# yungselm/multimoda-rs

Measured on AMD Instinct MI355X. Metric: Hausdorff pose-evals/sec (frames x poses) for 4-phase full align; best-pose match, higher is better.
Workload: dtype f16 hi+lo matrix-pipe screen (fp32 accumulate) + f64 exact re-score

## Files before the change

### multimoda-rs_amd/csrc/mm_kernels.hip

```cpp

#include <hip/hip_runtime.h>
#include <algorithm>
#include <cstdlib>
#include <type_traits>
#include <vector>
#include <cstdio>

#include "mm_device.h"
#include "mm_screen_limits.h"
#include "mm_xcd.h"
#include "../../include/mm_hausdorff.h"

namespace mm {

typedef float v2f __attribute__((ext_vector_type(2)));

template <typename T> struct Tr;
template <> struct Tr<float> {
    using U = unsigned int;
    using T2 = float2;
    static __device__ __forceinline__ U bits(float v) { return __float_as_uint(v); }
    static __device__ __forceinline__ float from(U u) { return __uint_as_float(u); }
    static __device__ __forceinline__ float inf() { return __uint_as_float(0x7f800000u); }
    static constexpr U INF_BITS = 0x7f800000u;
// ... 477 lines not shown
        }
    }
}


typedef _Float16 h2v __attribute__((ext_vector_type(2)));
typedef float f2v __attribute__((ext_vector_type(2)));

static __device__ __forceinline__ h4v mx_col_coords(float X, float Y)
{
    asm volatile("" : "+v"(X), "+v"(Y));
    h2v h = __builtin_convertvector(f2v{X, Y}, h2v);
    unsigned hb = __builtin_bit_cast(unsigned, h);
    asm volatile("" : "+v"(hb));
    h = __builtin_bit_cast(h2v, hb);
    const h2v l = __builtin_convertvector(f2v{X - (float)h.x, Y - (float)h.y}, h2v);
    return h4v{h.x, h.y, l.x, l.y};
}

static __device__ __forceinline__ h4v mx_col_norm(float X, float Y)
{
    const float n2 = __builtin_fmaf(X, X, Y * Y);
    const _Float16 nh = (_Float16)(n2 * 0.00390625f);
    const _Float16 nl = (_Float16)__builtin_fmaf(-256.0f, (float)nh, n2);
    return h4v{(_Float16)256.0f, (_Float16)1.0f, nh, nl};
}

template <int CTRL>
static __device__ __forceinline__ int dpp_max_i32(int v)
{
    const int o = __builtin_amdgcn_update_dpp((int)0x80000000, v, CTRL, 0xF, 0xF, false);
    return o > v ? o : v;
}
static __device__ __forceinline__ int wave_max_i32_dpp(int v)
{
    v = dpp_max_i32<0xB1>(v); v = dpp_max_i32<0x4E>(v); v = dpp_max_i32<0x141>(v); v = dpp_max_i32<0x140>(v);
    const int r0 = __builtin_amdgcn_readlane(v, 0), r1 = __builtin_amdgcn_readlane(v, 16);
    const int r2 = __builtin_amdgcn_readlane(v, 32), r3 = __builtin_amdgcn_readlane(v, 48);
    const int a = r0 > r1 ? r0 : r1, c = r2 > r3 ? r2 : r3;
    return a > c ? a : c;
}

#ifndef MM_MX_DUAL_MAX
#define MM_MX_DUAL_MAX 5
#endif
template <int NCT, bool CARRY>
static __device__ __forceinline__ int mx_main(unsigned vB, unsigned vA, unsigned vRW, unsigned vRR, int nloop, int tail, unsigned vRS)
{
    if constexpr (NCT <= MM_MX_DUAL_MAX) return MxMainD<NCT, CARRY>::run(vB, vA, nloop, tail, vRS);
    else return MxMain<NCT, CARRY>::run(vB, vA, vRW, vRR, 0u, nloop, tail, vRS);
}
template <int NCT>
static __device__ __forceinline__ int mx_emit(unsigned vB, unsigned vA, unsigned vRW, unsigned vRR, int nloop, int tail, unsigned vRS,
                                              unsigned vCS)
{
    if constexpr (NCT <= MM_MX_DUAL_MAX) return MxEmitD<NCT>::run(vB, vA, nloop, tail, vRS, vCS);
    else return MxEmit<NCT>::run(vB, vA, vRW, vRR, 0u, nloop, tail, vRS, vCS);
}

static __device__ __forceinline__ unsigned wave_min_u32_dpp(unsigned v)
{
    return ~(unsigned)wave_max_i32_dpp((int)~(v ^ 0x80000000u)) ^ 0x80000000u;
}

template <int NCT, bool MULTI, int WAVES = 4>
__global__ void __launch_bounds__(64 * WAVES, 2)
k_screen_mx(const PairDesc* __restrict__ pairs, const WorkItem* __restrict__ work, int n_work_host,
            const int* __restrict__ n_work_dev, const int32_t* __restrict__ sel, int a_cap, const float* __restrict__ ptx,
            const float* __restrict__ pty, const float* __restrict__ cosv, const float* __restrict__ sinv, float* __restrict__ out_sq)
{
    constexpr int NB = NCT * 32;
    constexpr int NQ = (NCT + 1) / 2;
    extern __shared__ __align__(16) unsigned char smem[];
    h8v* s_a = reinterpret_cast<h8v*>(smem);
    h4v* s_bw = reinterpret_cast<h4v*>(s_a + a_cap * 64);
    int* s_redx = reinterpret_cast<int*>(s_bw + WAVES * NCT * 64);
    int* s_rsx = s_redx + WAVES * MX_RED;
    float* s_cs = reinterpret_cast<float*>(s_rsx + (MULTI ? WAVES * a_cap * 32 : 0));
    int* s_ci = reinterpret_cast<int*>(s_cs + 2 * MX_ITEM);

    const int tid = threadIdx.x, lane = tid & 63, wave = tid >> 6, l32 = lane & 31, hi = lane >> 5;
    h4v* s_b = s_bw + wave * NCT * 64;
    int* s_rs = s_rsx + wave * a_cap * 32;
    const unsigned lds0 = (unsigned)(size_t)smem;
    const unsigned vB = lds0 + (unsigned)((size_t)s_b - (size_t)smem) + lane * 8;
    const unsigned vA = lds0 + (unsigned)((size_t)s_a - (size_t)smem) + lane * 16;
    const unsigned red_w = lds0 + (unsigned)((size_t)s_redx - (size_t)smem) + wave * MX_RED * 4;
    const unsigned vRW = red_w + (hi * 16) * MM_SCREEN_MX_RED_STRIDE + l32 * 4;
    const int rh = (l32 >> 2) & 1, rv = (l32 & 3) + 4 * (l32 >> 3);
    const unsigned vRR = red_w + (rh * 16 + rv) * MM_SCREEN_MX_RED_STRIDE + hi * 64;
    const unsigned vRS = lds0 + (unsigned)((size_t)s_rs - (size_t)smem) + l32 * 4;
    const int n_work = n_work_dev ? *n_work_dev : n_work_host;

    for (int wi = (int)gridDim.x == n_work ? xcd_work_index(blockIdx.x, n_work) : (int)blockIdx.x; wi < n_work;
         wi += gridDim.x) {
        const WorkItem w = work[wi];
        const PairDesc pd = pairs[w.pair];
        const int na = pd.n_ref, nb = pd.n_tgt;
        const int nrt = (na + 31) >> 5;
        const int nloop = (nrt - 1) >> 1, tail = (nrt - 1) & 1;
        const float S = __builtin_ldexpf(1.0f, pd.pad0), inv_s2 = __builtin_ldexpf(1.0f, -2 * pd.pad0);

        __syncthreads();
        for (int t = tid; t < 2 * w.cnt; t += 64 * WAVES) {
            const int a = sel ? sel[pd.out_off + w.a0 + (t >> 1)] : w.a0 + (t >> 1);
            s_cs[t] = (t & 1) ? sinv[pd.tab_off + a] : cosv[pd.tab_off + a];
            if (!(t & 1)) s_ci[t >> 1] = a;
        }
        mx_stage_rows<64 * WAVES>(s_a, nrt, na, ptx + pd.ref_off, pty + pd.ref_off, S, tid);
        if constexpr (!MULTI) {
            float tx[NQ], ty[NQ];
#pragma unroll
            for (int q = 0; q < NQ; ++q) {
                const int j = lane + 64 * q;
                const int jc = j < nb ? j : nb - 1;
                tx[q] = S * ptx[pd.tgt_off + jc]; ty[q] = S * pty[pd.tgt_off + jc];
                if (j < NB) s_b[(j >> 5) * 64 + (j & 31) + 32] = mx_col_norm(tx[q], ty[q]);
            }
            __syncthreads();

            for (int k = wave; k < w.cnt; k += WAVES) {
                const float c = s_cs[2 * k], s = s_cs[2 * k + 1];
                const int a = s_ci[k];
#pragma unroll
                for (int q = 0; q < NQ; ++q) {
                    const int j = lane + 64 * q;
                    if (j < NB) {
                        const float bx = __builtin_fmaf(tx[q], c, -(ty[q] * s));
                        const float by = __builtin_fmaf(tx[q], s, ty[q] * c);
                        s_b[(j >> 5) * 64 + (j & 31)] = mx_col_coords(bx, by);
                    }
                }
                int m = mx_main<NCT, false>(vB, vA, vRW, vRR, nloop, tail, vRS);
                m = wave_max_i32_dpp(m);
                if (lane == 0) out_sq[pd.out_off + a] = __int_as_float(m) * inv_s2;
            }
        } else {
            __syncthreads();
            const int nblk = (((nb + 31) >> 5) + NCT - 1) / NCT;
            for (int k = wave; k < w.cnt; k += WAVES) {
                const float c = s_cs[2 * k], s = s_cs[2 * k + 1];
                const int a = s_ci[k];
                for (int i = lane; i < nrt * 32; i += 64) s_rs[i] = 0x7f800000;
                int m = 0;
                for (int blk = 0; blk < nblk; ++blk) {
#pragma unroll
                    for (int q = 0; q < NQ; ++q) {
                        const int j = lane + 64 * q;
                        if (j < NB) {
                            const int jg = blk * NB + j;
                            const int jc = jg < nb ? jg : nb - 1;
                            const float x = S * ptx[pd.tgt_off + jc], y = S * pty[pd.tgt_off + jc];
                            const float bx = __builtin_fmaf(x, c, -(y * s));
                            const float by = __builtin_fmaf(x, s, y * c);
                            s_b[(j >> 5) * 64 + (j & 31) + 32] = mx_col_norm(x, y);
                            s_b[(j >> 5) * 64 + (j & 31)] = mx_col_coords(bx, by);
                        }
                    }
                    const int mb = mx_main<NCT, true>(vB, vA, vRW, vRR, nloop, tail, vRS);
                    m = mb > m ? mb : m;
                }
                for (int i = lane; i < nrt * 32; i += 64) { const int r = s_rs[i]; m = r > m ? r : m; }
                m = wave_max_i32_dpp(m);
                if (lane == 0) out_sq[pd.out_off + a] = __int_as_float(m) * inv_s2;
            }
        }
    }
}

template <int NCT>
__global__ void __launch_bounds__(64, 2)
k_screen_mx_emit(const PairDesc* __restrict__ pairs, const WorkItem* __restrict__ work, const int* __restrict__ n_work_dev, int a_cap,
                 const float* __restrict__ ptx, const float* __restrict__ pty, const float* __restrict__ cosv,
                 const float* __restrict__ sinv, float* __restrict__ out_sq, float* __restrict__ emit, int emit_rows, int emit_cols)
{
    constexpr int NB = NCT * 32, NQ = (NCT + 1) / 2;
    extern __shared__ __align__(16) unsigned char smem[];
    h8v* s_a = reinterpret_cast<h8v*>(smem);
    h4v* s_b = reinterpret_cast<h4v*>(s_a + a_cap * 64);
    int* s_red = reinterpret_cast<int*>(s_b + NCT * 64);
    int* s_rs = s_red + MX_RED;
    int* s_col = s_rs + a_cap * 32;
    const int lane = threadIdx.x, l32 = lane & 31, hi = lane >> 5;
    const unsigned lds0 = (unsigned)(size_t)smem;
    const unsigned vB = lds0 + (unsigned)((size_t)s_b - (size_t)smem) + lane * 8;
    const unsigned vA = lds0 + lane * 16;
    const unsigned red_w = lds0 + (unsigned)((size_t)s_red - (size_t)smem);
    const unsigned vRW = red_w + (hi * 16) * MM_SCREEN_MX_RED_STRIDE + l32 * 4;
    const int rh = (l32 >> 2) & 1, rv = (l32 & 3) + 4 * (l32 >> 3);
    const unsigned vRR = red_w + (rh * 16 + rv) * MM_SCREEN_MX_RED_STRIDE + hi * 64;
    const unsigned vRS = lds0 + (unsigned)((size_t)s_rs - (size_t)smem) + l32 * 4;
    const unsigned vCS = lds0 + (unsigned)((size_t)s_col - (size_t)smem) + lane * 4;
    const int n_work = *n_work_dev;

    for (int wi = blockIdx.x; wi < n_work; wi += gridDim.x) {
        const WorkItem w = work[wi];
        const PairDesc pd = pairs[w.pair];
        const int na = pd.n_ref, nb = pd.n_tgt, a = w.a0;
        const int nrt = (na + 31) >> 5, nloop = (nrt - 1) >> 1, tail = (nrt - 1) & 1;
        const float S = __builtin_ldexpf(1.0f, pd.pad0), inv_s2 = __builtin_ldexpf(1.0f, -2 * pd.pad0);
        const float c = cosv[pd.tab_off + a], s = sinv[pd.tab_off + a];
        __syncthreads();
        mx_stage_rows<64>(s_a, nrt, na, ptx + pd.ref_off, pty + pd.ref_off, S, lane);
        for (int i = lane; i < nrt * 32; i += 64) s_rs[i] = 0x7f800000;
#pragma unroll
        for (int q = 0; q < NQ; ++q) {
            const int j = lane + 64 * q;
            if (j < NB) {
                const int jc = j < nb ? j : nb - 1;
                const float x = S * ptx[pd.tgt_off + jc], y = S * pty[pd.tgt_off + jc];
                s_b[(j >> 5) * 64 + (j & 31) + 32] = mx_col_norm(x, y);
                s_b[(j >> 5) * 64 + (j & 31)] = mx_col_coords(__builtin_fmaf(x, c, -(y * s)), __builtin_fmaf(x, s, y * c));
            }
        }
        __syncthreads();
        int m = mx_emit<NCT>(vB, vA, vRW, vRR, nloop, tail, vRS, vCS);
        __syncthreads();
        float* const em = emit + (size_t)w.pair * (size_t)(emit_rows + emit_cols);
        for (int i = lane; i < nrt * 32; i += 64) {
            const int r = s_rs[i];
            m = r > m ? r : m;
            if (i < na) em[i] = __int_as_float(r) * inv_s2;
        }
        for (int j = lane; j < nb; j += 64) em[emit_rows + j] = __int_as_float(s_col[j]) * inv_s2;
        m = wave_max_i32_dpp(m);
        if (lane == 0) out_sq[pd.out_off + a] = __int_as_float(m) * inv_s2;
    }
}

template <int NCT>
static hipError_t launch_mx_emit_t(const BatchDev& b, const WorkItem* work, const int* n_dev, int cap, int a_cap, hipStream_t s)
{
    const size_t lds = (size_t)a_cap * 64 * 16 + (size_t)NCT * 64 * 8 + (size_t)MX_RED * 4 + (size_t)a_cap * 32 * 4 +
                       (size_t)((NCT + 1) / 2) * 64 * 4;
    hipError_t e = hipFuncSetAttribute(reinterpret_cast<const void*>(k_screen_mx_emit<NCT>), hipFuncAttributeMaxDynamicSharedMemorySize, (int)lds);
    if (e != hipSuccess) return e;
    hipLaunchKernelGGL((k_screen_mx_emit<NCT>), dim3(std::min(cap, 256 * 8 * 2)), dim3(64), lds, s, b.pairs, work, n_dev, a_cap, b.p32x,
                       b.p32y, b.cos32, b.sin32, b.sq32, b.emit, b.emit_rows, b.emit_cols);
    return hipGetLastError();
}

static hipError_t launch_mx_emit(const BatchDev& b, const WorkItem* work, const int* n_dev, int cap, int nct, int a_cap, hipStream_t s)
{
    if (a_cap < 1 || a_cap > 17) return hipErrorInvalidValue;
#define MM_MXE(N) case N: return launch_mx_emit_t<N>(b, work, n_dev, cap, a_cap, s);
    switch (nct) {
        MM_MXE(2) MM_MXE(3) MM_MXE(4) MM_MXE(5) MM_MXE(6) MM_MXE(7) MM_MXE(8) MM_MXE(9) MM_MXE(10) MM_MXE(11) MM_MXE(12) MM_MXE(13)
        MM_MXE(14) MM_MXE(15) MM_MXE(16) MM_MXE(17)
        default: return hipErrorInvalidValue;
    }
#undef MM_MXE
}

template <int NCT, bool MULTI>
static hipError_t launch_mx_t(const BatchDev& b, const WorkItem* work, int n_work, const int* n_dev, int cap, int a_cap, int waves,
                              const int32_t* sel, hipStream_t s)
{
    if constexpr (!MULTI) {
        if (waves == 1) {
            const size_t lds = lds_bytes_mx(NCT, false, a_cap, 1);
            hipError_t e = hipFuncSetAttribute(reinterpret_cast<const void*>(k_screen_mx<NCT, false, 1>), hipFuncAttributeMaxDynamicSharedMemorySize, (int)lds);
            if (e != hipSuccess) return e;
            const int grid = n_dev ? std::min(cap, 256 * 8 * 2) : n_work;
            hipLaunchKernelGGL((k_screen_mx<NCT, false, 1>), dim3(grid), dim3(64), lds, s, b.pairs, work, n_work, n_dev, sel, a_cap,
                               b.p32x, b.p32y, b.cos32, b.sin32, b.sq32);
            return hipGetLastError();
        }
    }
    const size_t lds = lds_bytes_mx(NCT, MULTI, a_cap, 4);
    hipError_t e = hipFuncSetAttribute(reinterpret_cast<const void*>(k_screen_mx<NCT, MULTI>), hipFuncAttributeMaxDynamicSharedMemorySize, (int)lds);
    if (e != hipSuccess) return e;
    const int grid = n_dev ? std::min(cap, 256 * 8) : n_work;
    hipLaunchKernelGGL((k_screen_mx<NCT, MULTI>), dim3(grid), dim3(256), lds, s, b.pairs, work, n_work, n_dev, sel, a_cap, b.p32x, b.p32y,
                       b.cos32, b.sin32, b.sq32);
    return hipGetLastError();
}

static hipError_t launch_mx_any(const BatchDev& b, const WorkItem* w, int n_work, const int* n_dev, int cap, int nct, int multi, int a_cap,
                                hipStream_t s, int waves = 4, const int32_t* sel = nullptr)
{
    if (a_cap < 1 || a_cap > MX_ROW_TILES_MAX || lds_bytes_mx(nct, multi != 0, a_cap, 4) > 160 * 1024) return hipErrorInvalidValue;
#define MM_MX(N) case N: return multi ? launch_mx_t<(N < 9 ? 9 : N), true>(b, w, n_work, n_dev, cap, a_cap, 4, sel, s) \
                                      : launch_mx_t<N, false>(b, w, n_work, n_dev, cap, a_cap, waves, sel, s);
    if (multi && nct < 9) return hipErrorInvalidValue;
    switch (nct) {
        MM_MX(2) MM_MX(3) MM_MX(4) MM_MX(5) MM_MX(6) MM_MX(7) MM_MX(8) MM_MX(9) MM_MX(10) MM_MX(11) MM_MX(12) MM_MX(13)
        MM_MX(14) MM_MX(15) MM_MX(16) MM_MX(17)
        default: return hipErrorInvalidValue;
    }
#undef MM_MX
}

hipError_t launch_screen_mx(const BatchDev& b, int work_begin, int n_work, int nct, int multi, int a_cap, hipStream_t s)
{
    if (n_work <= 0) return hipSuccess;
    return launch_mx_any(b, b.work + work_begin, n_work, nullptr, 0, nct, multi, a_cap, s);
}

typedef float f16x16 __attribute__((ext_vector_type(16)));

static constexpr int MXC_ROW_TILES_MAX = kMxCullRowTilesMax;
static constexpr int MXC_SETBIT_MIN_NCT = kMxCullSetbitMinNct;

static __device__ __forceinline__ int min3i(int a, int b, int c) { return min(a, min(b, c)); }

static __device__ __forceinline__ int mxc_fold(int acc, const f16x16& d)
{
    const int a0 = min3i(__float_as_int(d[0]), __float_as_int(d[1]), __float_as_int(d[2]));
    const int a1 = min3i(__float_as_int(d[3]), __float_as_int(d[4]), __float_as_int(d[5]));
    const int a2 = min3i(__float_as_int(d[6]), __float_as_int(d[7]), __float_as_int(d[8]));
    const int a3 = min3i(__float_as_int(d[9]), __float_as_int(d[10]), __float_as_int(d[11]));
    const int a4 = min3i(__float_as_int(d[12]), __float_as_int(d[13]), __float_as_int(d[14]));
    acc = min3i(acc, a0, a1);
    acc = min3i(acc, a2, a3);
    return min3i(acc, a4, __float_as_int(d[15]));
}

static __device__ __forceinline__ int mxc_meet(int v)
{
    const auto r = __builtin_amdgcn_permlane32_swap((unsigned)v, (unsigned)v, false, false);
    return min((int)r[0], (int)r[1]);
}

static __device__ __forceinline__ int half_max_i32_dpp(int v)
{
    v = dpp_max_i32<0xB1>(v); v = dpp_max_i32<0x4E>(v); v = dpp_max_i32<0x141>(v); v = dpp_max_i32<0x140>(v);
    const int r0 = __builtin_amdgcn_readlane(v, 0), r1 = __builtin_amdgcn_readlane(v, 16);
    return r0 > r1 ? r0 : r1;
}

#define MXC_MARK(s) __asm__ volatile("; mxc:" s)
#define MXC_MARK_V(s, x) __asm__ volatile("; mxc:" s : "+v"(x))

template <int N> struct mxc_regs {
    typedef int vec __attribute__((ext_vector_type(N - 1)));
    struct type {
        vec v;
        int last;
        __device__ __forceinline__ int get(int t) const { return t < N - 1 ? v[t] : last; }
        __device__ __forceinline__ void set(int t, int x) { if (t < N - 1) v[t] = x; else last = x; }
    };
};
typedef int mxc_i4 __attribute__((ext_vector_type(4)));

static __device__ __forceinline__ void mxc_tile(const h8v& af, int lo, int hi, int& c, int& rmin)
{
    const f16x16 z = {};
    const h8v b = __builtin_bit_cast(h8v, mxc_i4{lo, hi, lo, hi});
    const f16x16 d = __builtin_amdgcn_mfma_f32_32x32x16_f16(af, b, z, 0, 0, 0);
    const f16x16 e = __builtin_amdgcn_mfma_f32_32x32x16_f16(b, af, z, 0, 0, 0);
    __builtin_amdgcn_sched_barrier(0);
    c = mxc_fold(c, d);
    rmin = mxc_fold(rmin, e);
}

static __device__ __forceinline__ void mxc_tile2(const h8v& af, int loX, int hiX, int& cX, int& rminX, int loY, int hiY, int& cY,
                                                 int& rminY)
{
    const f16x16 z = {};
    const h8v bX = __builtin_bit_cast(h8v, mxc_i4{loX, hiX, loX, hiX});
    const h8v bY = __builtin_bit_cast(h8v, mxc_i4{loY, hiY, loY, hiY});
    const f16x16 dX = __builtin_amdgcn_mfma_f32_32x32x16_f16(af, bX, z, 0, 0, 0);
    const f16x16 eX = __builtin_amdgcn_mfma_f32_32x32x16_f16(bX, af, z, 0, 0, 0);
    __builtin_amdgcn_sched_barrier(0);
    cX = mxc_fold(cX, dX);
    __builtin_amdgcn_sched_barrier(0);
    const f16x16 dY = __builtin_amdgcn_mfma_f32_32x32x16_f16(af, bY, z, 0, 0, 0);
    __builtin_amdgcn_sched_barrier(0);
    rminX = mxc_fold(rminX, eX);
    __builtin_amdgcn_sched_barrier(0);
    const f16x16 eY = __builtin_amdgcn_mfma_f32_32x32x16_f16(bY, af, z, 0, 0, 0);
    __builtin_amdgcn_sched_barrier(0);
    cY = mxc_fold(cY, dY);
    rminY = mxc_fold(rminY, eY);
}

template <int NCT, int PH>
static __device__ __forceinline__ void mxc_tiles(unsigned mask, const h8v& af, const typename mxc_regs<NCT>::type& blo,
                                                 const typename mxc_regs<NCT>::type& bhi, typename mxc_regs<NCT>::type& cm, int& rmin)
{
    const unsigned tail = mask >> (NCT - 1);
    mask &= (1u << (NCT - 1)) - 1;
    while (mask) {
        MXC_MARK("tloop:tiles");
        const int t = __builtin_ctz(mask);
        mask &= mask - 1;
        const int lo = blo.v[t], hi = bhi.v[t];
        int c = cm.v[t];
        MXC_MARK_V("tile", c);
        mxc_tile(af, lo, hi, c, rmin);
        MXC_MARK_V("tloop:tiles", c);
        cm.v[t] = c;
    }
    if (tail) {
        MXC_MARK("tilet:tails");
        mxc_tile(af, blo.last, bhi.last, cm.last, rmin);
    }
    if constexpr (PH == 1) MXC_MARK_V("p1_row:lrows", rmin);
    else if constexpr (PH == 3) MXC_MARK_V("p1f_row:frows", rmin);
    else MXC_MARK_V("p2_row:rows2", rmin);
}

template <int NCT>
static __device__ __forceinline__ void mxc_tiles2(unsigned mask, const h8v& af, const typename mxc_regs<NCT>::type& bloX,
                                                  const typename mxc_regs<NCT>::type& bhiX, typename mxc_regs<NCT>::type& cmX, int& rminX,
                                                  const typename mxc_regs<NCT>::type& bloY, const typename mxc_regs<NCT>::type& bhiY,
                                                  typename mxc_regs<NCT>::type& cmY, int& rminY)
{
    const unsigned tail = mask >> (NCT - 1);
    mask &= (1u << (NCT - 1)) - 1;
    while (mask) {
        MXC_MARK("tloop2:ptiles");
        const int t = __builtin_ctz(mask);
        mask &= mask - 1;
        const int loX = bloX.v[t], hiX = bhiX.v[t], loY = bloY.v[t], hiY = bhiY.v[t];
        int cX = cmX.v[t], cY = cmY.v[t];
        MXC_MARK_V("tile2:ptiles", cX);
        mxc_tile2(af, loX, hiX, cX, rminX, loY, hiY, cY, rminY);
        MXC_MARK_V("tloop2:ptiles", cY);
        cmX.v[t] = cX;
        cmY.v[t] = cY;
    }
    if (tail) {
        MXC_MARK("tile2t:ptails");
        mxc_tile2(af, bloX.last, bhiX.last, cmX.last, rminX, bloY.last, bhiY.last, cmY.last, rminY);
    }
    MXC_MARK_V("p1p_row:prows", rminY);
}

template <int NCT, int PH>
static __device__ __forceinline__ void mxc_tiles_chain(unsigned mask, const h8v& af, const h4v (&bh)[NCT], int (&cm)[NCT], int& rmin)
{
    const f16x16 z = {};
#pragma unroll
    for (int t = 0; t < NCT; ++t) {
        if ((mask >> t) & 1) {
            MXC_MARK("tile");
            const h4v v = bh[t];
            const h8v b = h8v{v[0], v[1], v[2], v[3], v[0], v[1], v[2], v[3]};
            const f16x16 d = __builtin_amdgcn_mfma_f32_32x32x16_f16(af, b, z, 0, 0, 0);
            const f16x16 e = __builtin_amdgcn_mfma_f32_32x32x16_f16(b, af, z, 0, 0, 0);
            __builtin_amdgcn_sched_barrier(0);
            cm[t] = mxc_fold(cm[t], d);
            rmin = mxc_fold(rmin, e);
            if constexpr (PH == 1) MXC_MARK("p1_row:nrt"); else MXC_MARK("p2_row:rows2");
        }
    }
}

template <int NCT>
__global__ void __launch_bounds__(256, 2)
k_screen_mx_cull(const PairDesc* __restrict__ pairs, const WorkItem* __restrict__ work, int n_work,
                 const WorkRun* __restrict__ runs, int n_runs, int a_cap,
                 const float* __restrict__ ptx, const float* __restrict__ pty, const float* __restrict__ cosv,
                 const float* __restrict__ sinv, float* __restrict__ out_sq, unsigned long long* __restrict__ tiles_done,
                 int pair_on, int floor_on)
{
    constexpr int WAVES = 4, NB = NCT * 32, NQ = (NCT + 1) / 2, VS = 128, VM = 40, NT4 = (NCT + 3) / 4, NP = (NCT + 1) / 2;
    typedef typename mxc_regs<NCT>::type regs_t;
    extern __shared__ __align__(16) unsigned char smem[];
    h8v* s_a = reinterpret_cast<h8v*>(smem);
    h4v* s_bw = reinterpret_cast<h4v*>(s_a + a_cap * 64);
    int* s_rsx = reinterpret_cast<int*>(s_bw + WAVES * NCT * 64);
    float* s_thx = reinterpret_cast<float*>(s_rsx + WAVES * a_cap * 32);
    float4* s_circ = reinterpret_cast<float4*>(s_thx + WAVES * a_cap * 32);
    float* s_cs = reinterpret_cast<float*>(s_circ + NCT + a_cap);
    int* s_ci = reinterpret_cast<int*>(s_cs + 2 * MX_ITEM);
    int* s_ryx = s_ci + MX_ITEM;

    const int tid = threadIdx.x, lane = tid & 63, wave = tid >> 6, l32 = lane & 31;
    h4v* s_b = s_bw + wave * NCT * 64;
    int* s_rs = s_rsx + wave * a_cap * 32;
    int* s_ry = s_ryx + wave * a_cap * 32;
    (void)s_ry; (void)pair_on; (void)floor_on;
    float* s_th = s_thx + wave * a_cap * 32;
    int* s_v = reinterpret_cast<int*>(s_b);
    unsigned long long done = 0;
    unsigned n_foll = 0, n_early = 0;

    const int n_blocks = runs ? n_runs : n_work;
    for (int bi = runs ? (int)blockIdx.x : (int)gridDim.x == n_work ? xcd_work_index(blockIdx.x, n_work) : (int)blockIdx.x; bi < n_blocks;
         bi += gridDim.x) {
      int wi0 = bi, wi1 = bi + 1;
      if (runs) { const WorkRun r = runs[bi]; wi0 = r.first; wi1 = r.first + r.count; }
      int nrt = 0, tab_off = 0, out_off = 0;
      float inv_s2 = 0.0f, e2s = 0.0f;
      float tx[NQ], ty[NQ];
      for (int wi = wi0; wi < wi1; ++wi) {
        MXC_MARK("pro_item:item");
        const WorkItem w = work[wi];
        if (wi == wi0) { const PairDesc& pd0 = pairs[w.pair]; tab_off = pd0.tab_off; out_off = pd0.out_off; }

        __syncthreads();
        for (int t = tid; t < 2 * w.cnt; t += 64 * WAVES) {
            const int a = w.a0 + (t >> 1);
            s_cs[t] = (t & 1) ? sinv[tab_off + a] : cosv[tab_off + a];
            if (!(t & 1)) s_ci[t >> 1] = a;
        }
        if (wi == wi0) {
        MXC_MARK("pro_run:run");
        const PairDesc pd = pairs[w.pair];
        const int na = pd.n_ref, nb = pd.n_tgt;
        nrt = (na + 31) >> 5;
        const float S = __builtin_ldexpf(1.0f, pd.pad0);
        inv_s2 = __builtin_ldexpf(1.0f, -2 * pd.pad0);
        e2s = mm_tile_e2s(pd.e2, pd.pad0);
        mx_stage_rows<64 * WAVES>(s_a, nrt, na, ptx + pd.ref_off, pty + pd.ref_off, S, tid, pd.ref_main);
        MXC_MARK("pro_run:run");
#pragma unroll
        for (int q = 0; q < NQ; ++q) {
            const int j = lane + 64 * q;
            const int jc = mm_tile_slot_point(j, nb, pd.tgt_main);
            tx[q] = S * ptx[pd.tgt_off + jc]; ty[q] = S * pty[pd.tgt_off + jc];
            if (j < NB) s_b[(j >> 5) * 64 + (j & 31) + 32] = mx_col_norm(tx[q], ty[q]);
        }
        MXC_MARK("pro_run:run");
        if (tid < NCT) {
            float cx, cy, r;
            MXC_MARK("pro_run:run");
            mm_tile_circle(ptx + pd.tgt_off, pty + pd.tgt_off, tid * 32, nb, S, &cx, &cy, &r, pd.tgt_main);
            MXC_MARK("pro_run:run");
            s_circ[tid] = float4{cx, cy, r, 0.0f};
        } else if (tid >= 64 && tid < 64 + nrt) {
            float cx, cy, r;
            MXC_MARK("pro_run:run");
            mm_tile_circle(ptx + pd.ref_off, pty + pd.ref_off, (tid - 64) * 32, na, S, &cx, &cy, &r, pd.ref_main);
            MXC_MARK("pro_run:run");
            s_circ[NCT + tid - 64] = float4{cx, cy, r, 0.0f};
        }
        MXC_MARK("pro_item:item");
        }
        __syncthreads();
        MXC_MARK("end:0");
        const int G = NCT >= MXC_SETBIT_MIN_NCT ? min(max(w.pad, 1), 8) : 1;
        for (int k0 = wave * G; k0 < w.cnt; k0 += WAVES * G) {
          const int k1 = min(k0 + G, w.cnt);
          unsigned m1 = 0;
          int grp_tr = 0x7f800000;
          int grp_tc = 0x7f800000;
          unsigned grp_p1 = 0;
          if constexpr (NCT >= MXC_SETBIT_MIN_NCT) {
            MXC_MARK("thr:group");
            const int hw = lane >> 5;
            const bool jok = l32 < NCT;
            float4 cc = s_circ[jok ? l32 : NCT - 1];
            float cbx, cby;
            mm_tile_group_circle(cc.x, cc.y, cc.z, s_cs + 2 * k0, k1 - k0, &cbx, &cby, &cc.z);
            float ckey = __builtin_inff();
            int cbi = 0;
            float4 rc = s_circ[NCT + (hw < nrt ? hw : nrt - 1)];
            for (int p = 0; 2 * p < nrt; ++p) {
                MXC_MARK("thr_pass:ghalf");
                const int I = 2 * p + hw;
                const float4 rn = s_circ[NCT + (I + 2 < nrt ? I + 2 : nrt - 1)];
                const bool ok = jok && I < nrt;
                const float t = mm_tile_threshold(mm_tile_gap(rc.x, rc.y, rc.z, cbx, cby, cc.z), e2s);
                if (ok) s_th[I * 32 + l32] = t;
                const bool close = ok && !(t > 0.0f);
                const unsigned long long bal = __builtin_amdgcn_ballot_w64(close);
                m1 = lane == 2 * p ? (unsigned)bal : lane == 2 * p + 1 ? (unsigned)(bal >> 32) : m1;
                if (close) ckey = -1.0f;
                else if (ok && t < ckey) { ckey = t; cbi = I; }
                rc = rn;
            }
            MXC_MARK("m1:group");
            __asm__ volatile("" ::: "memory");
            if (lane < nrt && !m1) {
                const float4* q = reinterpret_cast<const float4*>(s_th + lane * 32);
                float th[NT4 * 4];
#pragma unroll
                for (int u = 0; u < NT4; ++u) { const float4 w4 = q[u]; th[4 * u] = w4.x; th[4 * u + 1] = w4.y; th[4 * u + 2] = w4.z; th[4 * u + 3] = w4.w; }
                float best = __builtin_inff();
                int bj = 0;
#pragma unroll
                for (int J = 0; J < NCT; ++J)
                    if (th[J] < best) { best = th[J]; bj = J; }
                m1 = 1u << bj;
            }
            int lone_i = -1;
            {
                const auto kk = __builtin_amdgcn_permlane32_swap((unsigned)__float_as_int(ckey), (unsigned)__float_as_int(ckey), false, false);
                const auto ii = __builtin_amdgcn_permlane32_swap((unsigned)cbi, (unsigned)cbi, false, false);
                const float key0 = __int_as_float((int)kk[0]), key1 = __int_as_float((int)kk[1]);
                const int i0 = (int)ii[0], i1 = (int)ii[1];
                if (lane < NCT && key0 > 0.0f && key1 > 0.0f) lone_i = key1 < key0 ? i1 : key1 == key0 ? min(i0, i1) : i0;
            }
            for (unsigned long long lone = __builtin_amdgcn_ballot_w64(lone_i >= 0); lone; lone &= lone - 1) {
                const int L = __builtin_ctzll(lone), I = __builtin_amdgcn_readlane(lone_i, L);
                if (lane == I) m1 |= 1u << L;
            }
            if (floor_on) {
                MXC_MARK("flr_tr:group");
                if (lane < nrt) {
                    const float4* q = reinterpret_cast<const float4*>(s_th + lane * 32);
                    float th[NT4 * 4];
#pragma unroll
                    for (int u = 0; u < NT4; ++u) { const float4 w4 = q[u]; th[4 * u] = w4.x; th[4 * u + 1] = w4.y; th[4 * u + 2] = w4.z; th[4 * u + 3] = w4.w; }
                    int tr = 0x7f800000;
#pragma unroll
                    for (int J = 0; J < NCT; ++J)
                        if (!((m1 >> J) & 1)) tr = min(tr, __float_as_int(th[J]));
                    grp_tr = tr;
                }
                int tc = 0x7f800000;
                for (int p = 0; 2 * p < nrt; ++p) {
                    MXC_MARK("flr_tc_row:ghalf");
                    const int I1 = min(2 * p + 1, nrt - 1);
                    const unsigned pm0 = __builtin_amdgcn_readlane(m1, 2 * p), pm1 = __builtin_amdgcn_readlane(m1, I1);
                    const int t = __float_as_int(s_th[(hw ? I1 : 2 * p) * 32 + l32]);
                    if (!(((hw ? pm1 : pm0) >> l32) & 1)) tc = min(tc, t);
                }
                MXC_MARK("flr_tr:group");
                grp_tc = mxc_meet(tc);
            }
          }
          (void)m1; (void)grp_tr; (void)grp_tc; (void)grp_p1;
          for (int k = k0; k < k1; ++k) {
            const float c = s_cs[2 * k], s = s_cs[2 * k + 1];
            const int a = s_ci[k];
            if constexpr (NCT >= MXC_SETBIT_MIN_NCT) {
                const bool follower = __builtin_amdgcn_readfirstlane(k > k0) != 0;
                const bool paired = __builtin_amdgcn_readfirstlane(pair_on && k > k0 && k + 1 < k1) != 0;
                MXC_MARK("setup:xcand");
                auto stage_cols = [&](float c, float s, regs_t& blo, regs_t& bhi) {
#pragma unroll
                    for (int q = 0; q < NQ; ++q) {
                        const int j = lane + 64 * q;
                        if (j < NB) {
                            const float bx = __builtin_fmaf(tx[q], c, -(ty[q] * s));
                            const float by = __builtin_fmaf(tx[q], s, ty[q] * c);
                            s_b[(j >> 5) * 64 + (j & 31)] = mx_col_coords(bx, by);
                        }
                    }
                    __asm__ volatile("" ::: "memory");
#pragma unroll
                    for (int t = 0; t < NCT; ++t) {
                        const int2 v = reinterpret_cast<const int2*>(s_b)[t * 64 + lane];
                        blo.set(t, v.x); bhi.set(t, v.y);
                    }
                    __asm__ volatile("" ::: "memory");
                };
                regs_t blo, bhi;
                stage_cols(c, s, blo, bhi);

                MXC_MARK("p1_init:xcand");
                const unsigned p1m = m1;
                regs_t cm;
#pragma unroll
                for (int t = 0; t < NCT; ++t) cm.set(t, 0x7f800000);
                h8v af = s_a[lane];
                int fmax = 0;
                unsigned long long late = 0;
                const bool upper = lane >= 32;
                auto p1_rows = [&](auto fol) {
                    for (int I = 0; I < nrt; ++I) {
                        constexpr bool FOL = decltype(fol)::value;
                        if constexpr (FOL) MXC_MARK("p1f_row:frows"); else MXC_MARK("p1_row:lrows");
                        const unsigned mask = __builtin_amdgcn_readlane(p1m, I);
                        const h8v an = s_a[(I + 1 < nrt ? I + 1 : I) * 64 + lane];
                        int rmin = 0x7f800000;
                        mxc_tiles<NCT, FOL ? 3 : 1>(mask, af, blo, bhi, cm, rmin);
                        rmin = mxc_meet(rmin);
                        if (lane < 32) s_rs[I * 32 + lane] = rmin;
                        const bool above = rmin > __builtin_amdgcn_readlane(grp_tr, I);
                        if constexpr (FOL) {
                            fmax = max(fmax, above && upper ? 0 : rmin);
                            late |= __builtin_amdgcn_ballot_w64(above);
                        } else {
                            fmax = max(fmax, above ? 0 : rmin);
                            done += __builtin_popcount(mask);
                        }
                        af = an;
                    }
                };
                auto fol_check = [&](const regs_t& cmf, int& fm, unsigned long long& lt, int& lo) {
                    __builtin_amdgcn_sched_barrier(0);
#pragma unroll
                    for (int p = 0; p < NP; ++p) {
                        const int c0 = cmf.get(2 * p), c1 = cmf.get(2 * p + 1 < NCT ? 2 * p + 1 : 2 * p);
                        const auto r = __builtin_amdgcn_permlane32_swap((unsigned)c0, (unsigned)c1, false, false);
                        const int v = min((int)r[0], (int)r[1]);
                        const int t0 = __builtin_amdgcn_readlane(grp_tc, 2 * p), t1 = __builtin_amdgcn_readlane(grp_tc, 2 * p + 1 < NCT ? 2 * p + 1 : 2 * p);
                        const bool above = v > (lane < 32 ? t0 : t1);
                        lt |= __builtin_amdgcn_ballot_w64(above);
                        fm = max(fm, v);
                        lo = max(lo, above ? 0 : v);
                    }
                };
                auto fol_leaves = [&](int fm, unsigned long long lt, int lo, int ai, int& L) -> bool {
                    done += grp_p1;
                    ++n_foll;
                    const int F = wave_max_i32_dpp(fm);
                    L = floor_on ? wave_max_i32_dpp(lo) : (int)0x80000000;
                    const bool leaves = floor_on ? F <= L : lt == 0;
                    if (leaves) {
                        ++n_early;
                        if (lane == 0) out_sq[out_off + ai] = __int_as_float(F) * inv_s2;
                    }
                    return leaves;
                };
                unsigned stay = 1;
                int LX = (int)0x80000000, LY = (int)0x80000000;
                regs_t bloY, bhiY, cmY;
                int aY = a;
                if (paired) {
                    MXC_MARK("setup2:pair");
                    aY = s_ci[k + 1];
                    stage_cols(s_cs[2 * k + 2], s_cs[2 * k + 3], bloY, bhiY);
                    MXC_MARK("p1_init2:pair");
#pragma unroll
                    for (int t = 0; t < NCT; ++t) cmY.set(t, 0x7f800000);
                    int fmaxY = 0;
                    unsigned long long lateY = 0;
                    for (int I = 0; I < nrt; ++I) {
                        MXC_MARK("p1p_row:prows");
                        const unsigned mask = __builtin_amdgcn_readlane(p1m, I);
                        const int tr = __builtin_amdgcn_readlane(grp_tr, I);
                        const h8v an = s_a[(I + 1 < nrt ? I + 1 : I) * 64 + lane];
                        int rminX = 0x7f800000, rminY = 0x7f800000;
                        mxc_tiles2<NCT>(mask, af, blo, bhi, cm, rminX, bloY, bhiY, cmY, rminY);
                        rminX = mxc_meet(rminX);
                        rminY = mxc_meet(rminY);
                        if (lane < 32) { s_rs[I * 32 + lane] = rminX; s_ry[I * 32 + lane] = rminY; }
                        const bool aboveX = rminX > tr, aboveY = rminY > tr;
                        late |= __builtin_amdgcn_ballot_w64(aboveX);
                        lateY |= __builtin_amdgcn_ballot_w64(aboveY);
                        fmax = max(fmax, aboveX && upper ? 0 : rminX);
                        fmaxY = max(fmaxY, aboveY && upper ? 0 : rminY);
                        af = an;
                    }
                    MXC_MARK("fol_check2:pair");
                    int flo = upper ? fmax : 0, floY = upper ? fmaxY : 0;
                    fol_check(cm, fmax, late, flo);
                    fol_check(cmY, fmaxY, lateY, floY);
                    const bool goX = fol_leaves(fmax, late, flo, a, LX), goY = fol_leaves(fmaxY, lateY, floY, aY, LY);
                    stay = (goX ? 0u : 1u) | (goY ? 0u : 2u);
                    MXC_MARK("end:0");
                } else {
                    if (follower) p1_rows(std::true_type{}); else p1_rows(std::false_type{});
                    if (follower) {
                        MXC_MARK("fol_check:sfol");
                        int flo = upper ? fmax : 0;
                        fol_check(cm, fmax, late, flo);
                        if (fol_leaves(fmax, late, flo, a, LX)) stay = 0;
                        MXC_MARK("end:0");
                    } else if (floor_on) {
                        MXC_MARK("flr_lead:lead");
                        int flo = fmax;
                        fol_check(cm, fmax, late, flo);
                        LX = wave_max_i32_dpp(flo);
                        MXC_MARK("end:0");
                    }
                    __asm__ volatile("" : "=v"(bloY.v), "=v"(bhiY.v), "=v"(cmY.v), "=v"(bloY.last), "=v"(bhiY.last), "=v"(cmY.last));
                }
                int acur = a;
                int* rs = s_rs;
                for (; stay; stay &= stay - 1) {
                if (!(stay & 1)) {
                    MXC_MARK("ymove:ylate");
                    blo = bloY; bhi = bhiY; cm = cmY;
                    acur = aY; rs = s_ry; LX = LY;
                }
                MXC_MARK("vmax:late");
#pragma unroll
                for (int t = 0; t < NCT; ++t) {
                    cm.set(t, mxc_meet(cm.get(t)));
                    if (lane < 32) s_v[t * VS + lane] = cm.get(t);
                }
                __asm__ volatile("" ::: "memory");
                if (lane < NCT) {
                    const int4* q = reinterpret_cast<const int4*>(s_v + lane * VS);
                    int v = (int)0x80000000;
#pragma unroll
                    for (int u = 0; u < 8; ++u) { const int4 w4 = q[u]; v = max(v, max(max(w4.x, w4.y), max(w4.z, w4.w))); }
                    s_v[VM + lane] = v > LX ? v : (int)0x80000000;
                }
                __asm__ volatile("" ::: "memory");
                MXC_MARK("m2:late");
                unsigned m2 = 0;
                int rowmax = 0;
                const bool leads = !follower && __builtin_amdgcn_readfirstlane(k1 - k0) > 1;
                if (lane < nrt) {
                    const int4* q = reinterpret_cast<const int4*>(rs + lane * 32);
                    int umax = (int)0x80000000;
#pragma unroll
                    for (int u = 0; u < 8; ++u) { const int4 w4 = q[u]; umax = max(umax, max(max(w4.x, w4.y), max(w4.z, w4.w))); }
                    const int ulive = umax > LX ? umax : (int)0x80000000;
                    const float4* qt = reinterpret_cast<const float4*>(s_th + lane * 32);
                    const int4* qv = reinterpret_cast<const int4*>(s_v + VM);
                    float th[NT4 * 4];
                    int vm[NT4 * 4];
#pragma unroll
                    for (int u = 0; u < NT4; ++u) {
                        const float4 w4 = qt[u]; th[4 * u] = w4.x; th[4 * u + 1] = w4.y; th[4 * u + 2] = w4.z; th[4 * u + 3] = w4.w;
                        const int4 v4 = qv[u]; vm[4 * u] = v4.x; vm[4 * u + 1] = v4.y; vm[4 * u + 2] = v4.z; vm[4 * u + 3] = v4.w;
                    }
#pragma unroll
                    for (int J = 0; J < NCT; ++J) {
                        const float t = th[J];
                        const int lim = max(ulive, vm[J]);
                        if (!(t > 0.0f && __float_as_int(t) >= lim)) m2 |= 1u << J;
                    }
                    m2 &= ~p1m;
                    if (!m2) rowmax = umax;
                    if (leads) {
                        MXC_MARK("grp_tr:fgroup");
                        const unsigned pf = p1m | m2;
                        int tr = 0x7f800000;
#pragma unroll
                        for (int J = 0; J < NCT; ++J)
                            if (!((pf >> J) & 1)) tr = min(tr, __float_as_int(th[J]));
                        grp_tr = tr;
                        MXC_MARK("m2:late");
                    }
                }
                if (!follower) m1 |= m2;
                if (leads) {
                    MXC_MARK("grp_tc:fgroup");
                    const unsigned pf = m1;
                    int tc = 0x7f800000;
                    unsigned cnt = 0;
                    for (int p = 0; 2 * p < nrt; ++p) {
                        MXC_MARK("grp_tc_row:fghalf");
                        const int I1 = min(2 * p + 1, nrt - 1);
                        const unsigned pm0 = __builtin_amdgcn_readlane(pf, 2 * p), pm1 = __builtin_amdgcn_readlane(pf, I1);
                        const int t = __float_as_int(s_th[(upper ? I1 : 2 * p) * 32 + l32]);
                        if (!(((upper ? pm1 : pm0) >> l32) & 1)) tc = min(tc, t);
                        cnt += __builtin_popcount(pm0) + (2 * p + 1 < nrt ? __builtin_popcount(pm1) : 0);
                    }
                    MXC_MARK("grp_tc:fgroup");
                    grp_tc = mxc_meet(tc);
                    grp_p1 = cnt;
                }

                for (unsigned long long rows = __builtin_amdgcn_ballot_w64(m2 != 0); rows; rows &= rows - 1) {
                    MXC_MARK("p2_row:rows2");
                    const int I = __builtin_ctzll(rows);
                    const unsigned mask = __builtin_amdgcn_readlane(m2, I);
                    const h8v ai = s_a[I * 64 + lane];
                    int rmin = rs[I * 32 + l32];
                    mxc_tiles<NCT, 2>(mask, ai, blo, bhi, cm, rmin);
                    rmin = mxc_meet(rmin);
                    done += __builtin_popcount(mask);
                    rowmax = max(rowmax, rmin);
                }
                MXC_MARK("final:late");
                int m = rowmax;
#pragma unroll
                for (int t = 0; t < NCT; ++t) m = max(m, mxc_meet(cm.get(t)));
                m = wave_max_i32_dpp(m);
                if (lane == 0) out_sq[out_off + acur] = __int_as_float(m) * inv_s2;
                MXC_MARK("end:0");
                }
                if (paired) ++k;
            } else {
                MXC_MARK("setup:1");
#pragma unroll
                for (int q = 0; q < NQ; ++q) {
                    const int j = lane + 64 * q;
                    if (j < NB) {
                        const float bx = __builtin_fmaf(tx[q], c, -(ty[q] * s));
                        const float by = __builtin_fmaf(tx[q], s, ty[q] * c);
                        s_b[(j >> 5) * 64 + (j & 31)] = mx_col_coords(bx, by);
                    }
                }
                __asm__ volatile("" ::: "memory");
                h4v bf[NCT];
#pragma unroll
                for (int t = 0; t < NCT; ++t) bf[t] = s_b[t * 64 + lane];
                __asm__ volatile("" ::: "memory");

                MXC_MARK("thr:1");
                for (int p = lane; p < nrt * NCT; p += 64) {
                    MXC_MARK("thr_pass:pairs64");
                    const int I = p / NCT, J = p - I * NCT;
                    const float4 rc = s_circ[NCT + I], cc = s_circ[J];
                    const float bx = __builtin_fmaf(cc.x, c, -(cc.y * s)), by = __builtin_fmaf(cc.x, s, cc.y * c);
                    s_th[I * 32 + J] = mm_tile_threshold(mm_tile_gap(rc.x, rc.y, rc.z, bx, by, cc.z), e2s);
                }
                __asm__ volatile("" ::: "memory");
                MXC_MARK("m1:1");
                unsigned m1 = 0;
                int lone_i = -1;
                if (lane < nrt) {
                    float best = __builtin_inff();
                    int bj = 0;
#pragma unroll
                    for (int J = 0; J < NCT; ++J) {
                        const float t = s_th[lane * 32 + J];
                        if (!(t > 0.0f)) m1 |= 1u << J;
                        if (t < best) { best = t; bj = J; }
                    }
                    if (!m1) m1 = 1u << bj;
                } else if (lane >= 32 && lane - 32 < NCT) {
                    const int J = lane - 32;
                    bool cov = false;
                    float best = __builtin_inff();
                    int bi = 0;
                    for (int I = 0; I < nrt; ++I) {
                        MXC_MARK("lone_loop:nrt");
                        const float t = s_th[I * 32 + J];
                        cov = cov || !(t > 0.0f);
                        if (t < best) { best = t; bi = I; }
                    }
                    MXC_MARK("m1:1");
                    lone_i = cov ? -1 : bi;
                }
                for (unsigned long long lone = __builtin_amdgcn_ballot_w64(lone_i >= 0); lone; lone &= lone - 1) {
                    const int L = __builtin_ctzll(lone), I = __builtin_amdgcn_readlane(lone_i, L);
                    if (lane == I) m1 |= 1u << (L - 32);
                }

                MXC_MARK("p1_init:1");
                int cm[NCT];
#pragma unroll
                for (int t = 0; t < NCT; ++t) cm[t] = 0x7f800000;
                h8v af = s_a[lane];
                for (int I = 0; I < nrt; ++I) {
                    MXC_MARK("p1_row:nrt");
                    const unsigned mask = __builtin_amdgcn_readlane(m1, I);
                    const h8v an = s_a[(I + 1 < nrt ? I + 1 : I) * 64 + lane];
                    int rmin = 0x7f800000;
                    mxc_tiles_chain<NCT, 1>(mask, af, bf, cm, rmin);
                    rmin = mxc_meet(rmin);
                    if (lane < 32) s_rs[I * 32 + lane] = rmin;
                    done += __builtin_popcount(mask);
                    af = an;
                }
                MXC_MARK("vmax:1");
#pragma unroll
                for (int t = 0; t < NCT; ++t) {
                    cm[t] = mxc_meet(cm[t]);
                    if (lane < 32) s_v[t * VS + lane] = cm[t];
                }
                __asm__ volatile("" ::: "memory");
                if (lane < NCT) {
                    const int4* q = reinterpret_cast<const int4*>(s_v + lane * VS);
                    int v = (int)0x80000000;
#pragma unroll
                    for (int u = 0; u < 8; ++u) { const int4 w4 = q[u]; v = max(v, max(max(w4.x, w4.y), max(w4.z, w4.w))); }
                    s_v[lane * VS + 40] = v;
                }
                __asm__ volatile("" ::: "memory");
                MXC_MARK("m2:1");
                unsigned m2 = 0;
                int rowmax = 0;
                if (lane < nrt) {
                    const int4* q = reinterpret_cast<const int4*>(s_rs + lane * 32);
                    int umax = (int)0x80000000;
#pragma unroll
                    for (int u = 0; u < 8; ++u) { const int4 w4 = q[u]; umax = max(umax, max(max(w4.x, w4.y), max(w4.z, w4.w))); }
#pragma unroll
                    for (int J = 0; J < NCT; ++J) {
                        const float t = s_th[lane * 32 + J];
                        const int lim = max(umax, s_v[J * VS + 40]);
                        if (!(t > 0.0f && __float_as_int(t) >= lim)) m2 |= 1u << J;
                    }
                    m2 &= ~m1;
                    if (!m2) rowmax = umax;
                }

                for (unsigned long long rows = __builtin_amdgcn_ballot_w64(m2 != 0); rows; rows &= rows - 1) {
                    MXC_MARK("p2_row:rows2");
                    const int I = __builtin_ctzll(rows);
                    const unsigned mask = __builtin_amdgcn_readlane(m2, I);
                    const h8v ai = s_a[I * 64 + lane];
                    int rmin = s_rs[I * 32 + l32];
                    mxc_tiles_chain<NCT, 2>(mask, ai, bf, cm, rmin);
                    rmin = mxc_meet(rmin);
                    done += __builtin_popcount(mask);
                    rowmax = max(rowmax, rmin);
                }
                MXC_MARK("final:1");
                int m = rowmax;
#pragma unroll
                for (int t = 0; t < NCT; ++t) m = max(m, mxc_meet(cm[t]));
                m = wave_max_i32_dpp(m);
                if (lane == 0) out_sq[out_off + a] = __int_as_float(m) * inv_s2;
                MXC_MARK("end:0");
            }
          }
        }
      }
    }
    if (tiles_done && lane == 0 && done) {
        atomicAdd(tiles_done, done);
        if (n_foll) { atomicAdd(tiles_done + 1, (unsigned long long)n_early); atomicAdd(tiles_done + 2, (unsigned long long)n_foll); }
    }
}

template <int NCT>
static hipError_t launch_mx_cull_t(const BatchDev& b, const WorkItem* work, int n_work, const WorkRun* runs, int n_runs, int a_cap,
                                   unsigned long long* tiles, int pair, int floor, hipStream_t s)
{
    const size_t lds = lds_bytes_mx_cull(NCT, a_cap);
    hipError_t e = hipFuncSetAttribute(reinterpret_cast<const void*>(k_screen_mx_cull<NCT>), hipFuncAttributeMaxDynamicSharedMemorySize, (int)lds);
    if (e != hipSuccess) return e;
    hipLaunchKernelGGL((k_screen_mx_cull<NCT>), dim3(runs ? n_runs : n_work), dim3(256), lds, s, b.pairs, work, n_work, runs, n_runs,
                       a_cap, b.p32x, b.p32y, b.cos32, b.sin32, b.sq32, tiles, pair, floor);
    return hipGetLastError();
}

hipError_t launch_screen_mx_cull(const BatchDev& b, int work_begin, int n_work, const WorkRun* runs, int n_runs, int nct, int a_cap,
                                 unsigned long long* tiles, int pair, int floor, hipStream_t s)
{
    if (n_work <= 0) return hipSuccess;
    if (!mx_cull_takes(nct, 0, a_cap) || (runs && n_runs <= 0)) return hipErrorInvalidValue;
    if (!runs) n_runs = 0;
    const WorkItem* w = b.work + work_begin;
#define MM_MXC(N) case N: return launch_mx_cull_t<N>(b, w, n_work, runs, n_runs, a_cap, tiles, pair, floor, s);
    switch (nct) {
        MM_MXC(2) MM_MXC(3) MM_MXC(4) MM_MXC(5) MM_MXC(6) MM_MXC(7) MM_MXC(8) MM_MXC(9) MM_MXC(10) MM_MXC(11) MM_MXC(12)
        MM_MXC(13) MM_MXC(14) MM_MXC(15) MM_MXC(16) MM_MXC(17)
        default: return hipErrorInvalidValue;
    }
#undef MM_MXC
}

static constexpr int kLbRP = kLbRowPairs;

static __device__ __forceinline__ float fmin3_f32(float a, float b, float c)
{
    float r;
    asm("v_min3_f32 %0, %1, %2, %3" : "=v"(r) : "v"(a), "v"(b), "v"(c));
    return r;
}

template <int RP>
static __device__ __forceinline__ int lb_pass(const v2f (&qx)[RP], const v2f (&qy)[RP], const v2f (&q2)[RP],
                                              const float4* __restrict__ s_p, int n_groups, int lj)
{
    v2f rm[RP];
#pragma unroll
    for (int q = 0; q < RP; ++q) rm[q] = (v2f)(__int_as_float(0x7f800000));
    float4 p0 = s_p[lj], p1 = s_p[16 + lj];
    for (int k = 0; k < n_groups; k += 2) {
        const int kn = k + 2 < n_groups ? k + 2 : k;
        const float4 n0 = s_p[kn * 16 + lj];
// ... 1200 lines not shown
```

Before: 210.6 million.

## Pack paired X/Y reductions into wave halves via permlane32 swap and reschedule tile loads

In the paired follower path, the X and Y row minima are now combined with a single permlane32 swap, so the lower half of the wave holds X and the upper half holds Y. One ballot and one max/floor accumulator then serve both candidates, and the final column check and reductions are done once with DPP partial reductions that split per half. mxc_tile2 now issues the Y operand loads and accumulator reads after the X MFMAs through a callback, to overlap register fetches with matrix-pipe latency. The row-min store also drops its lane<32 predicate and writes from all lanes. Correctness depends on the lane-half mapping, on the s_rs/s_ry store aliasing, and on the late/floor semantics matching the old per-candidate logic.

```diff
diff --git a/multimoda-rs_amd/csrc/mm_kernels.hip b/multimoda-rs_amd/csrc/mm_kernels.hip
--- a/multimoda-rs_amd/csrc/mm_kernels.hip
+++ b/multimoda-rs_amd/csrc/mm_kernels.hip
@@ -803,7 +803,7 @@
 static constexpr int MXC_ROW_TILES_MAX = kMxCullRowTilesMax;
 static constexpr int MXC_SETBIT_MIN_NCT = kMxCullSetbitMinNct;
 
-static __device__ __forceinline__ int min3i(int a, int b, int c) { return min(a, min(b, c)); }
+static __device__ __forceinline__ int min3i(int a, int b, int c) { return min(min(a, b), c); }
 
 static __device__ __forceinline__ int mxc_fold(int acc, const f16x16& d)
 {
@@ -855,14 +855,16 @@
     rmin = mxc_fold(rmin, e);
 }
 
-static __device__ __forceinline__ void mxc_tile2(const h8v& af, int loX, int hiX, int& cX, int& rminX, int loY, int hiY, int& cY,
-                                                 int& rminY)
+template <class Rest>
+static __device__ __forceinline__ void mxc_tile2(const h8v& af, int loX, int hiX, int& cX, int& rminX, int& cY, int& rminY, Rest&& rest)
 {
     const f16x16 z = {};
     const h8v bX = __builtin_bit_cast(h8v, mxc_i4{loX, hiX, loX, hiX});
-    const h8v bY = __builtin_bit_cast(h8v, mxc_i4{loY, hiY, loY, hiY});
     const f16x16 dX = __builtin_amdgcn_mfma_f32_32x32x16_f16(af, bX, z, 0, 0, 0);
     const f16x16 eX = __builtin_amdgcn_mfma_f32_32x32x16_f16(bX, af, z, 0, 0, 0);
+    __builtin_amdgcn_sched_barrier(0);
+    h8v bY;
+    rest(bY, cX, cY);
     __builtin_amdgcn_sched_barrier(0);
     cX = mxc_fold(cX, dX);
     __builtin_amdgcn_sched_barrier(0);
@@ -914,17 +916,29 @@
         MXC_MARK("tloop2:ptiles");
         const int t = __builtin_ctz(mask);
         mask &= mask - 1;
-        const int loX = bloX.v[t], hiX = bhiX.v[t], loY = bloY.v[t], hiY = bhiY.v[t];
-        int cX = cmX.v[t], cY = cmY.v[t];
-        MXC_MARK_V("tile2:ptiles", cX);
-        mxc_tile2(af, loX, hiX, cX, rminX, loY, hiY, cY, rminY);
+        const int loX = bloX.v[t], hiX = bhiX.v[t];
+        int cX, cY;
+        MXC_MARK("tile2:ptiles");
+        mxc_tile2(af, loX, hiX, cX, rminX, cY, rminY, [&](h8v& bY, int& x, int& y) {
+            const int loY = bloY.v[t], hiY = bhiY.v[t];
+            x = cmX.v[t]; y = cmY.v[t];
+            __builtin_amdgcn_sched_barrier(0);
+            bY = __builtin_bit_cast(h8v, mxc_i4{loY, hiY, loY, hiY});
+            __asm__("" : "+v"(bY));
+        });
         MXC_MARK_V("tloop2:ptiles", cY);
         cmX.v[t] = cX;
         cmY.v[t] = cY;
     }
     if (tail) {
         MXC_MARK("tile2t:ptails");
-        mxc_tile2(af, bloX.last, bhiX.last, cmX.last, rminX, bloY.last, bhiY.last, cmY.last, rminY);
+        int loX = bloX.last, hiX = bhiX.last;
+        __asm__ volatile("" : "+v"(loX), "+v"(hiX));
+        mxc_tile2(af, loX, hiX, cmX.last, rminX, cmY.last, rminY, [&](h8v& bY, int&, int&) {
+            int loY = bloY.last, hiY = bhiY.last;
+            __asm__ volatile("" : "+v"(loY), "+v"(hiY));
+            bY = __builtin_bit_cast(h8v, mxc_i4{loY, hiY, loY, hiY});
+        });
     }
     MXC_MARK_V("p1p_row:prows", rminY);
 }
@@ -1162,7 +1176,7 @@
                         int rmin = 0x7f800000;
                         mxc_tiles<NCT, FOL ? 3 : 1>(mask, af, blo, bhi, cm, rmin);
                         rmin = mxc_meet(rmin);
-                        if (lane < 32) s_rs[I * 32 + lane] = rmin;
+                        s_rs[I * 32 + l32] = rmin;
                         const bool above = rmin > __builtin_amdgcn_readlane(grp_tr, I);
                         if constexpr (FOL) {
                             fmax = max(fmax, above && upper ? 0 : rmin);
@@ -1188,17 +1202,19 @@
                         lo = max(lo, above ? 0 : v);
                     }
                 };
-                auto fol_leaves = [&](int fm, unsigned long long lt, int lo, int ai, int& L) -> bool {
+                auto fol_verdict = [&](int F, int Lw, bool late, int ai, int& L) -> bool {
                     done += grp_p1;
                     ++n_foll;
-                    const int F = wave_max_i32_dpp(fm);
-                    L = floor_on ? wave_max_i32_dpp(lo) : (int)0x80000000;
-                    const bool leaves = floor_on ? F <= L : lt == 0;
+                    L = floor_on ? Lw : (int)0x80000000;
+                    const bool leaves = floor_on ? F <= L : !late;
                     if (leaves) {
                         ++n_early;
                         if (lane == 0) out_sq[out_off + ai] = __int_as_float(F) * inv_s2;
                     }
                     return leaves;
+                };
+                auto fol_leaves = [&](int fm, unsigned long long lt, int lo, int ai, int& L) -> bool {
+                    return fol_verdict(wave_max_i32_dpp(fm), floor_on ? wave_max_i32_dpp(lo) : 0, lt != 0, ai, L);
                 };
                 unsigned stay = 1;
                 int LX = (int)0x80000000, LY = (int)0x80000000;
@@ -1211,8 +1227,9 @@
                     MXC_MARK("p1_init2:pair");
 #pragma unroll
                     for (int t = 0; t < NCT; ++t) cmY.set(t, 0x7f800000);
-                    int fmaxY = 0;
-                    unsigned long long lateY = 0;
+                    int fall = 0, fset = 0;
+                    unsigned long long lateXY = 0;
+                    int* const rsxy = upper ? s_ry : s_rs;
                     for (int I = 0; I < nrt; ++I) {
                         MXC_MARK("p1p_row:prows");
                         const unsigned mask = __builtin_amdgcn_readlane(p1m, I);
@@ -1220,21 +1237,37 @@
                         const h8v an = s_a[(I + 1 < nrt ? I + 1 : I) * 64 + lane];
                         int rminX = 0x7f800000, rminY = 0x7f800000;
                         mxc_tiles2<NCT>(mask, af, blo, bhi, cm, rminX, bloY, bhiY, cmY, rminY);
-                        rminX = mxc_meet(rminX);
-                        rminY = mxc_meet(rminY);
-                        if (lane < 32) { s_rs[I * 32 + lane] = rminX; s_ry[I * 32 + lane] = rminY; }
-                        const bool aboveX = rminX > tr, aboveY = rminY > tr;
-                        late |= __builtin_amdgcn_ballot_w64(aboveX);
-                        lateY |= __builtin_amdgcn_ballot_w64(aboveY);
-                        fmax = max(fmax, aboveX && upper ? 0 : rminX);
-                        fmaxY = max(fmaxY, aboveY && upper ? 0 : rminY);
+                        const auto r = __builtin_amdgcn_permlane32_swap((unsigned)rminX, (unsigned)rminY, false, false);
+                        const int rm = min((int)r[0], (int)r[1]);
+                        rsxy[I * 32 + l32] = rm;
+                        const bool above = rm > tr;
+                        lateXY |= __builtin_amdgcn_ballot_w64(above);
+                        fall = max(fall, rm);
+                        fset = max(fset, above ? 0 : rm);
                         af = an;
                     }
                     MXC_MARK("fol_check2:pair");
-                    int flo = upper ? fmax : 0, floY = upper ? fmaxY : 0;
-                    fol_check(cm, fmax, late, flo);
-                    fol_check(cmY, fmaxY, lateY, floY);
-                    const bool goX = fol_leaves(fmax, late, flo, a, LX), goY = fol_leaves(fmaxY, lateY, floY, aY, LY);
+                    __builtin_amdgcn_sched_barrier(0);
+#pragma unroll
+                    for (int t = 0; t < NCT; ++t) {
+                        const auto r = __builtin_amdgcn_permlane32_swap((unsigned)cm.get(t), (unsigned)cmY.get(t), false, false);
+                        const int v = min((int)r[0], (int)r[1]);
+                        const bool above = v > __builtin_amdgcn_readlane(grp_tc, t);
+                        lateXY |= __builtin_amdgcn_ballot_w64(above);
+                        fall = max(fall, v);
+                        fset = max(fset, above ? 0 : v);
+                        if (t % 4 == 3) __builtin_amdgcn_sched_barrier(0);
+                    }
+                    auto halves = [&](int v, int& x, int& y) {
+                        v = dpp_max_i32<0xB1>(v); v = dpp_max_i32<0x4E>(v); v = dpp_max_i32<0x141>(v); v = dpp_max_i32<0x140>(v);
+                        x = max(__builtin_amdgcn_readlane(v, 0), __builtin_amdgcn_readlane(v, 16));
+                        y = max(__builtin_amdgcn_readlane(v, 32), __builtin_amdgcn_readlane(v, 48));
+                    };
+                    int FX, FY, SX = 0, SY = 0;
+                    halves(fall, FX, FY);
+                    if (floor_on) halves(fset, SX, SY);
+                    const bool goX = fol_verdict(FX, SX, (unsigned)lateXY != 0, a, LX);
+                    const bool goY = fol_verdict(FY, SY, (lateXY >> 32) != 0, aY, LY);
                     stay = (goX ? 0u : 1u) | (goY ? 0u : 2u);
                     MXC_MARK("end:0");
                 } else {
```

Result: faster. 224.2 million, median of 6 (+6.4%).
